# vpc-ccg/freddie

Measured on AMD Instinct MI355X. Metric: reads segmented/sec (whole node), higher is better.
Workload: dtype u32

## Files before the change

### freddie_amd/csrc/seg_common.h

```cpp
#pragma once
#include <hip/hip_runtime.h>
#include <type_traits>
#include <hsa/hsa.h>
#include <hsa/hsa_ext_amd.h>
#include <chrono>
#include <algorithm>
#include <atomic>
#include <mutex>
#include <cmath>
#include <cstdarg>
#include <cstdio>
#include <cstdlib>
#include <cstring>
#include <string>
#include <vector>

#include "freddie_seg.h"

namespace fseg {


typedef long long i64;

typedef unsigned long long u64;
// ... 344 lines not shown
#define FSEG_VAL(x) (pass ? __dmul_rn(__dsub_rn((x), mu), __dsub_rn((x), mu)) : (x))
    for (int t0 = 0; t0 < nl; t0 += 64) {
        int t = t0 + (threadIdx.x >> 3);
        double res = 0.0;
        if (t < nl) {
            const double *b = a + L.leaf_off[t];
            int len = L.leaf_len[t];
            if (len < 8) {
                for (int i = 0; i < len; ++i) res = __dadd_rn(res, FSEG_VAL(b[i]));
            } else {
                int body = len - (len % 8);
                double x[16];
#pragma unroll
                for (int i = 0; i < 16; ++i) x[i] = (8 * i + q < body) ? b[8 * i + q] : 0.0;
                double r = FSEG_VAL(x[0]);
#pragma unroll
                for (int i = 1; i < 16; ++i) if (8 * i + q < body) r = __dadd_rn(r, FSEG_VAL(x[i]));
                r = __dadd_rn(r, __shfl_xor(r, 1));
                r = __dadd_rn(r, __shfl_xor(r, 2));
                r = __dadd_rn(r, __shfl_xor(r, 4));
                res = r;
                for (int i = body; i < len; ++i) res = __dadd_rn(res, FSEG_VAL(b[i]));
            }
        }
        if (t < nl && q == 0) L.node_val[L.leaf_heap[t]] = res;
    }
#undef FSEG_VAL
    __syncthreads();
    double out = 0.0;
    if (m == 8192) {
        if (threadIdx.x < 64) {
            double x = L.node_val[64 + threadIdx.x];
            for (int d = 1; d < 64; d <<= 1) x = __dadd_rn(x, __shfl_xor(x, d));
            out = x;
        }
    } else {
        for (int lvl = 6; lvl >= 0; --lvl) {
            const int i = (1 << lvl) + threadIdx.x;
            if ((int)threadIdx.x < (1 << lvl) && L.node_kind[i] == 2) L.node_val[i] = __dadd_rn(L.node_val[2 * i], L.node_val[2 * i + 1]);
            __syncthreads();
        }
        if (threadIdx.x == 0) out = L.node_val[1];
    }
    return out;
}

constexpr int kThrPartMaxChunks = 128;

__device__ __forceinline__ int wave_emit_values(i64 w0, i64 n_pos, unsigned fm, i64 ex, const double *__restrict__ y, double *v) {
    const int lane = lane_id();
    const u64 lt_mask = (1ULL << lane) - 1ULL;
    u64 rows;
    {
        const u64 lanes_set = __ballot(fm != 0);
        u64 pairs = (lanes_set | (lanes_set >> 1)) & 0x5555555555555555ULL;
        pairs = (pairs | (pairs >> 1)) & 0x3333333333333333ULL;
        pairs = (pairs | (pairs >> 2)) & 0x0f0f0f0f0f0f0f0fULL;
        pairs = (pairs | (pairs >> 4)) & 0x00ff00ff00ff00ffULL;
        pairs = (pairs | (pairs >> 8)) & 0x0000ffff0000ffffULL;
        rows = (pairs | (pairs >> 16)) & 0x00000000ffffffffULL;
    }
    int cnt = 0;
    while (rows) {
        u64 m[8];
        double yv[8];
#pragma unroll
        for (int e = 0; e < 8; ++e) {
            const int q = rows ? (int)__builtin_ctzll(rows) : -1;
            rows = rows ? rows & (rows - 1) : 0;
            const int qq = q < 0 ? 0 : q;
            const unsigned lo = (unsigned)__builtin_amdgcn_readlane((int)fm, 2 * qq);
            const unsigned hi = (unsigned)__builtin_amdgcn_readlane((int)fm, 2 * qq + 1);
            m[e] = q < 0 ? 0 : ((u64)lo | ((u64)hi << 32));
            const i64 i = w0 + qq * 64 + lane;
            yv[e] = y[i < n_pos ? i : n_pos - 1];
        }
#pragma unroll
        for (int e = 0; e < 8; ++e) {
            if (!m[e]) continue;
            if ((m[e] >> lane) & 1ULL) v[ex + cnt + __popcll(m[e] & lt_mask)] = yv[e];
            cnt += __popcll(m[e]);
        }
    }
    return cnt;
}


__device__ __forceinline__ void peak_from(i64 p, i64 last , const double *x, unsigned *flag) {
    const double xi = x[p];
    if (!(x[p - 1] < xi)) return;
    if (x[p + 1] < xi) { set_flag(flag, p); return; }
    if (x[p + 1] == xi) {
        i64 ia = p + 1;
        while (ia < last && x[ia] == xi) ++ia;
        if (x[ia] < xi) set_flag(flag, (p + ia - 1) / 2);
    }
}


struct ProblemArrays {
    int *iv;
    int *start;
    int *n;
    i64 *pair_off;
    i64 *tri_off;
    int *flags;
    int *chain;
    i64 *cov_off;
    int *lane_lo;
    int *lane_n;
};

struct __align__(16) ProbDesc {
    i64 c0;
    i64 pair_off, tri_off, cov_off;
    int n, lane_lo, lane_n;
    int g0;
    int outside;
    int iv;
    int w0;
    int kind;
};

static_assert(sizeof(ProbDesc) == 64, "ProbDesc is one 64-byte record");

__device__ __forceinline__ ProbDesc load_desc(const ProbDesc *d) {
    const uint4 *q = reinterpret_cast<const uint4 *>(d);
    union { uint4 v[4]; ProbDesc p; } u;
    u.v[0] = q[0]; u.v[1] = q[1]; u.v[2] = q[2]; u.v[3] = q[3];
    return u.p;
}


typedef int int4u __attribute__((ext_vector_type(4), aligned(4)));

typedef int int2u __attribute__((ext_vector_type(2), aligned(4)));

__device__ __forceinline__ void load_exons8(const int *p, int (&v)[8]) {
    const int4u a = *reinterpret_cast<const int4u *>(p), b = *reinterpret_cast<const int4u *>(p + 4);
    v[0] = a.x; v[1] = a.y; v[2] = a.z; v[3] = a.w; v[4] = b.x; v[5] = b.y; v[6] = b.z; v[7] = b.w;
}

__device__ __forceinline__ int2 load_exons2(const int *p) {
    const int2u a = *reinterpret_cast<const int2u *>(p);
    return make_int2(a.x, a.y);
}

constexpr size_t kExonPad = 32;

constexpr size_t kLexPad = 64;


__device__ __forceinline__ int uni(int v) { return __builtin_amdgcn_readfirstlane(v); }

__device__ __forceinline__ int wave_id() { return uni((int)(threadIdx.x >> 6)); }

__device__ __forceinline__ ProbDesc load_desc_uniform(const ProbDesc *d) {
    const uint4 *q = reinterpret_cast<const uint4 *>(d);
    union { uint4 v[4]; int w[16]; ProbDesc p; } u;
    u.v[0] = q[0]; u.v[1] = q[1]; u.v[2] = q[2]; u.v[3] = q[3];
#pragma unroll
    for (int i = 0; i < 16; ++i) u.w[i] = uni(u.w[i]);
    return u.p;
}


#ifdef FSEG_DESC_VECTOR
#define FSEG_LOAD_DESC load_desc
#else
#define FSEG_LOAD_DESC load_desc_uniform
#endif

__device__ __forceinline__ i64 wave_excl_scan(i64 v, i64 *total) {
    int lane = lane_id();
    i64 x = v;
    for (int d = 1; d < 64; d <<= 1) {
        i64 y = __shfl_up(x, d);
        if (lane >= d) x += y;
    }
    *total = __shfl(x, 63);
    return x - v;
}


__device__ __forceinline__ int wg_prev_flagged(bool f, int idx, int &carry, int *lds) {
    int lane = lane_id(), wave = threadIdx.x >> 6, nw = (blockDim.x + 63) >> 6;
    u64 mask = __ballot(f);
    __syncthreads();
    if (lane == 0) lds[wave] = mask ? idx + 63 - __clzll((long long)mask) : -1;
    __syncthreads();
    u64 below = mask & ((1ULL << lane) - 1ULL);
    int prev = carry;
    if (below) prev = idx - lane + 63 - __clzll((long long)below);
    else for (int w = wave - 1; w >= 0; --w) if (lds[w] >= 0) { prev = lds[w]; break; }
    for (int w = nw - 1; w >= 0; --w) if (lds[w] >= 0) { carry = lds[w]; break; }
    return prev;
}


__device__ __forceinline__ void window_exons(const int2 *__restrict__ lex, int2 lx, int cp0, int c_last, int *first_rel, int *cnt_out) {
    const int n_ex = lx.y - lx.x;
    int fr = 0, cnt = 0;
    for (int eb = 0; eb < n_ex; eb += 8) {
        int4u x[4];
#pragma unroll
        for (int u = 0; u < 4; ++u) x[u] = *reinterpret_cast<const int4u *>(lex + lx.x + eb + 2 * u);
#pragma unroll
        for (int u = 0; u < 4; ++u) {
            const bool hit0 = eb + 2 * u < n_ex && x[u].y >= cp0 && x[u].x < c_last;
            if (hit0 && cnt == 0) fr = eb + 2 * u;
            cnt += hit0;
            const bool hit1 = eb + 2 * u + 1 < n_ex && x[u].w >= cp0 && x[u].z < c_last;
            if (hit1 && cnt == 0) fr = eb + 2 * u + 1;
            cnt += hit1;
        }
        if (eb + 7 < n_ex && x[3].z >= c_last) break;
    }
    *first_rel = fr; *cnt_out = cnt;
}


constexpr int kRangeThreads = 1024;


constexpr int kProbCols = 9;

__device__ __forceinline__ i64 col_lo(i64 x) { return x & 0xffffffffLL; }

__device__ __forceinline__ i64 col_hi(i64 x) { return (i64)((u64)x >> 32); }

constexpr int kDpSmall = 32;

constexpr int kClsSmall = 16, kClsMid = 32;

struct ProbSizes { i64 v[kProbCols]; };

__device__ __forceinline__ int size_class(int n) { return n <= kClsSmall ? 0 : (n <= kClsMid ? 1 : (n <= kNMax ? 2 : 3)); }

struct ProbSplit { int tiny_max, fuse_lanes; };

enum { kKindArena = 0, kKindTiny = 1, kKindFused = 2, kKindFusedWide = 3 };

__device__ __forceinline__ int prob_kind(int n, int n_lanes, ProbSplit sp) {
    if (n <= sp.tiny_max) return kKindTiny;
    return (n_lanes <= sp.fuse_lanes && n <= kNMax) ? kKindFused : kKindArena;
}

__device__ __forceinline__ ProbSizes prob_sizes(int n, int n_lanes, ProbSplit sp) {
    ProbSizes s;
    for (int q = 0; q < kProbCols; ++q) s.v[q] = 0;
    if (n <= 0) return s;
    const int kind = prob_kind(n, n_lanes, sp);
    if (kind == kKindTiny) { s.v[0] = 1; s.v[8] = 1LL << 32; return s; }
    if (kind == kKindFused) {
        const int c = size_class(n);
        s.v[0] = 1;
        s.v[7] = c == 0 ? 1 : (c == 1 ? (1LL << 32) : 0);
        s.v[8] = c == 2 ? 1 : 0;
        return s;
    }
    i64 chunks = (n_lanes + kLaneChunk - 1) / kLaneChunk;
    const int cls = size_class(n);
    s.v[0] = 1 + (n <= kDpSmall ? (1LL << 32) : 0);
    s.v[1] = (i64)n * (n - 1) / 2; s.v[2] = (i64)n * (n - 1) * (n - 2) / 6;
    s.v[3] = chunks * kLaneChunk * n;
    s.v[4] = cls == 0 ? chunks : (cls == 1 ? chunks << 32 : 0);
    s.v[5] = (cls == 2 ? chunks : 0) + ((n > kDpSmall && n <= kNMax) ? (1LL << 32) : 0);
    s.v[6] = (cls == 3 ? chunks : 0) + (n > kNMax ? (1LL << 32) : 0);
    return s;
}

__device__ __forceinline__ i64 wg_exclusive_scan64(i64 v, i64 *lds , i64 *total) {
    int lane = lane_id(), wave = threadIdx.x >> 6, nw = (blockDim.x + 63) >> 6;
    i64 x = v;
    for (int d = 1; d < 64; d <<= 1) {
        i64 y = __shfl_up(x, d);
        if (lane >= d) x += y;
    }
    __syncthreads();
    if (lane == 63) lds[wave] = x;
    __syncthreads();
    i64 off = 0, tot = 0;
    for (int w = 0; w < nw; ++w) {
        i64 sv = lds[w];
        if (w < wave) off += sv;
        tot += sv;
    }
    *total = tot;
    return off + x - v;
}

constexpr int kProbBlock = 1024;

__device__ __forceinline__ void wg_scan_cols(const ProbSizes &v, ProbSizes &ex, ProbSizes &tot, i64 *lds ) {
    const int lane = lane_id(), wave = threadIdx.x >> 6;
    for (int q = 0; q < kProbCols; ++q) {
        i64 x = v.v[q];
        if (__ballot(x != 0)) {
            for (int d = 1; d < 64; d <<= 1) {
                i64 y = __shfl_up(x, d);
                if (lane >= d) x += y;
            }
        }
        ex.v[q] = x - v.v[q];
        if (lane == 63) lds[wave * kProbCols + q] = x;
    }
// ... 588 lines not shown
```

### freddie_amd/csrc/seg_score_fused.hip

```cpp
#include "seg_kernels.h"

namespace fseg {


#ifndef FSEG_TINY_OCC
#define FSEG_TINY_OCC 5
#endif
__global__ void __launch_bounds__(256, FSEG_TINY_OCC) k_tiny(Status *st, const ProbDesc *desc, i64 prob_cap, int tiny_max, ProblemArrays pr,
                                              const int *cand_y, const longlong2 *lane_ex, const int *ex_ts,
                                              const int *ex_te, const double *h_table, int h_len, double tau, const int2 *thr_tab,
                                              int support, unsigned char *chosen, i64 lb_h, i64 ln_h FSEG_TPARAM) {
    __shared__ u64 planes[4][kTinyPairs][2];
    __shared__ i64 M_s[4][kTinyPairs];
    __shared__ int in_s[4][kTinyPairs];
    __shared__ unsigned out_s[4][kTinyTri + 4];
    __shared__ unsigned char A_s[4][kTinyPairs + 4];
    __shared__ int cy_s[4][kTiny];
    __shared__ unsigned char tri_ijk[kTinyTri][4];
    __shared__ int2 act_w[4][128];
    const int lane = lane_id(), wave = wave_id();
    const u64 lt_mask = (1ULL << lane) - 1ULL;
    if (threadIdx.x < kTinyTri) {
        int t = threadIdx.x, k = 2;
        while ((k + 1) * k * (k - 1) / 6 <= t) ++k;
// ... 80 lines not shown
            int cov[kTiny];
#pragma unroll
            for (int j = 0; j < kTiny; ++j) cov[j] = 0;
            {
                const int2 a = act_w[wave][valid ? lane : 0];
                const int e_end = valid ? a.y : 0;
                for (int e = 0; e < e_end; e += 2) {
                    const int2 ts2 = load_exons2(ex_ts + a.x + e), te2 = load_exons2(ex_te + a.x + e);
                    const int tsa = ts2.x, tea = te2.x, tsb = ts2.y, teb = te2.y;
                    const int a0 = max(tsa, cp0), b0 = tea + 1;
                    const int a1 = max(tsb, cp0), b1 = e + 1 < e_end ? teb + 1 : a1;
#pragma unroll
                    for (int j = 1; j < kTiny; ++j) cov[j] += max(0, min(b0, cj[j]) - a0) + max(0, min(b1, cj[j]) - a1);
                }
            }
            const u64 vmask = __ballot(valid);
            u64 my_yea = 0, my_nay = 0;
#pragma unroll
            for (int j = 1; j < kTiny; ++j) {
#pragma unroll
                for (int i = 0; i < j; ++i) {
                    const int q = j * (j - 1) / 2 + i;
                    if (q < npairs) {
                        const int dd = cov[j] - cov[i];
                        const int hi = __builtin_amdgcn_readlane(hi_q, q), lo = __builtin_amdgcn_readlane(lo_q, q);
                        const u64 y = __ballot(valid && dd >= hi), z = __ballot(valid && dd <= lo);
                        if (lane == q) { my_yea = y; my_nay = z; }
                    }
                }
            }
            if (lane < npairs) {
                amb += (unsigned)__popcll(~(my_yea | my_nay) & vmask);
                planes[wave][lane][0] = my_yea; planes[wave][lane][1] = my_nay;
            }
            int2 keep = make_int2(0, 0);
            if (lane < fill - nv) keep = act_w[wave][64 + lane];
            dp_sync<64>();
            if (lane < fill - nv) act_w[wave][lane] = keep;
            fill -= nv;
            if (lane < ntri) {
                const int qa = tj * (tj - 1) / 2 + ti, qb = tk * (tk - 1) / 2 + tj;
                out += (unsigned)(__popcll(planes[wave][qa][0] & planes[wave][qb][1]) + __popcll(planes[wave][qa][1] & planes[wave][qb][0]));
            }
            dp_sync<64>();
        }
        const int dropped = d.lane_n - n_act;
        if (lane < npairs) in_s[wave][lane] = -(int)((i64)amb + (lo_q < 0 ? (i64)d.outside + dropped : 0));
        if (lane < ntri) out_s[wave][lane] = out;
        dp_sync<64>();
        const int chain = dp_solve_push<64, kTiny>(n, out_s[wave], in_s[wave], M_s[wave], A_s[wave], cy_s[wave], support, chosen + d.c0 FSEG_DARG);
        if (lane == 0) pr.chain[p] = chain;
#ifdef FSEG_SCORE_TIMING
        if (lane == 0) FSEG_PROB_TICK(p, t_prob0, d.lane_n, n_act);
#endif
    }
}

template <int NM, typename V>
__global__ void __launch_bounds__(256, WaveCfg<NM>::kOcc) k_wave(Status *st, const ProbDesc *desc, i64 prob_cap, int list, ProblemArrays pr,
                                                                 const int *__restrict__ cand_y, const int2 *__restrict__ lane_lx, const int2 *__restrict__ lex,
                                                                 const double *h_table, int h_len, double tau, const int2 *__restrict__ thr_tab,
                                                                 int support, unsigned char *chosen, i64 lb_h, i64 ln_h FSEG_TPARAM) {
    using C = WaveCfg<NM>;
    __shared__ WaveLds<NM, V> lds4[4];
    __shared__ unsigned short tri_q[C::kTri + 2];
    const int lane = lane_id(), wave = wave_id();
    WaveLds<NM, V> &L = lds4[wave];
    for (int t = threadIdx.x; t < C::kTri; t += 256) {
        int k = 2;
        while ((k + 1) * k * (k - 1) / 6 <= t) ++k;
        int i, j;
        pair_decode(t - k * (k - 1) * (k - 2) / 6, &i, &j);
        tri_q[t] = (unsigned short)((j * (j - 1) / 2 + i) | ((k * (k - 1) / 2 + j) << 8));
    }
    __syncthreads();
    if (lb_h < 0 && (i64)st->n_prob > prob_cap) return;
#ifdef FSEG_SCORE_TIMING
    __shared__ unsigned long long tick_sink[16];
    unsigned long long *dp_tacc = tick_sink; unsigned long long dt_prev = 0;
#endif
    const i64 list_base = lb_h >= 0 ? lb_h : (list == 3 ? (i64)st->solve_cls[0] + (i64)st->solve_cls[1] + (i64)st->solve_cls[2] : 0);
    const i64 list_n = lb_h >= 0 ? ln_h : (list == 3 ? (i64)st->n_tiny : (i64)st->solve_cls[0]);
    const unsigned aborted = stage_aborted(st);
    for (i64 t = (i64)blockIdx.x + (i64)wave * gridDim.x; t < list_n; t += (i64)gridDim.x * 4) {
#ifdef FSEG_SCORE_TIMING
        const unsigned long long t_prob0 = wall_clock64();
#endif
        const ProbDesc d = FSEG_LOAD_DESC(desc + list_base + t);
        if (aborted) return;
        const int p = d.w0;
        const int n = d.n;
        if (n > NM || n < 3) { if (lane == 0) atomicOr(&st->err, kErrOverflowNm); continue; }
        const int npairs = n * (n - 1) / 2, ntri = n * (n - 1) * (n - 2) / 6;
        int2 lx = lane_lx[d.lane_lo + (lane < d.lane_n ? lane : 0)];
        const int cyv = cand_y[d.c0 + (lane < n ? lane : 0)];
        dp_sync<64>();
        if (lane < n) L.cy[lane] = cyv;
        int hi_q[C::kPSlots], lo_q[C::kPSlots];
        unsigned amb[C::kPSlots], outc[C::kTSlots];
#pragma unroll
        for (int s = 0; s < C::kPSlots; ++s) {
            const int q = s * 64 + lane;
            hi_q[s] = 0x7fffffff; lo_q[s] = -1; amb[s] = 0;
            const unsigned short ij = g_pair_ij[q < npairs ? q : 0];
            const int ci = __shfl(cyv, ij & 255), cjv = __shfl(cyv, ij >> 8);
            if (q < npairs) label_thresholds_tab((i64)cjv - ci + 1, thr_tab, h_table, h_len, tau, &hi_q[s], &lo_q[s]);
        }
#pragma unroll
        for (int s = 0; s < C::kTSlots; ++s) outc[s] = 0;
        const int cp0 = d.g0 + __builtin_amdgcn_readlane(cyv, 0), c_last = d.g0 + __builtin_amdgcn_readlane(cyv, n - 1);
        int cj[NM];
#pragma unroll
        for (int j = 0; j < NM; ++j) cj[j] = j < n ? d.g0 + __builtin_amdgcn_readlane(cyv, j) : cp0;
        for (int l0 = 0; l0 < d.lane_n;) {
            const bool in = l0 + lane < d.lane_n;
            if (l0 > 0) lx = lane_lx[d.lane_lo + l0 + (in ? lane : 0)];
            const int base = uni(lx.x) & ~1;
            const u64 fm = __ballot(in && lx.y - base <= kStageCap);
            const int m = ~fm == 0 ? 64 : (int)__builtin_ctzll(~fm);
            if (m == 0) { if (lane == 0) atomicOr(&st->err, kErrWaveStage); break; }
            const int total = __builtin_amdgcn_readlane(lx.y, m - 1) - base;
            {
                const int last2 = total & ~1;
                int4 sv[kStageCap / 128];
#pragma unroll
                for (int u = 0; u < kStageCap / 128; ++u) {
                    const int i = 2 * lane + 128 * u;
                    sv[u] = *reinterpret_cast<const int4 *>(lex + base + (i < last2 ? i : last2));
                }
#pragma unroll
                for (int u = 0; u < kStageCap / 128; ++u) {
                    const int i = 2 * lane + 128 * u;
                    if (i < total) *reinterpret_cast<int4 *>(&L.stage[i]) = sv[u];
                }
            }
            dp_sync<64>();
            const bool valid = lane < m;
            const u64 vmask = m == 64 ? ~0ULL : ((1ULL << m) - 1ULL);
            const int ea = valid ? lx.x - base : 0, eb = valid ? lx.y - base : 0;
            int first = ea, cnt = 0;
            for (int e = ea; e < eb; e += 4) {
                int2 x[4];
#pragma unroll
                for (int u = 0; u < 4; ++u) x[u] = L.stage[e + u];
#pragma unroll
                for (int u = 0; u < 4; ++u) {
                    const bool hit = e + u < eb && x[u].y >= cp0 && x[u].x < c_last;
                    if (hit && cnt == 0) first = e + u;
                    cnt += hit;
                }
                if (x[3].x >= c_last) break;
            }
            int cov[NM];
#pragma unroll
            for (int j = 0; j < NM; ++j) cov[j] = 0;
            for (int e = 0; e < cnt; e += 2) {
                const int2 xa = L.stage[first + e], xb = L.stage[first + e + 1];
                const int a0 = max(xa.x, cp0), b0 = xa.y + 1;
                const int a1 = max(xb.x, cp0), b1 = e + 1 < cnt ? xb.y + 1 : a1;
#pragma unroll
                for (int j = 1; j < NM; ++j)
                    if (j < n) cov[j] += max(0, min(b0, cj[j]) - a0) + max(0, min(b1, cj[j]) - a1);
            }
            unsigned yl[C::kPSlots], yh[C::kPSlots], zl[C::kPSlots], zh[C::kPSlots];
#pragma unroll
            for (int s = 0; s < C::kPSlots; ++s) { yl[s] = 0; yh[s] = 0; zl[s] = 0; zh[s] = 0; }
            static_for<1, NM>([&](auto jc) {
                constexpr int j = decltype(jc)::value;
                if (j < n) {
                    static_for<0, j>([&](auto ic) {
                        constexpr int i = decltype(ic)::value;
                        constexpr int q = j * (j - 1) / 2 + i, s = q >> 6, ql = q & 63;
                        const int dd = cov[j] - cov[i];
                        const int hi = __builtin_amdgcn_readlane(hi_q[s], ql), lo = __builtin_amdgcn_readlane(lo_q[s], ql);
                        const u64 y = __ballot(dd >= hi) & vmask, z = __ballot(dd <= lo) & vmask;
                        write_lane<ql>(yl[s], (unsigned)y); write_lane<ql>(yh[s], (unsigned)(y >> 32));
                        write_lane<ql>(zl[s], (unsigned)z); write_lane<ql>(zh[s], (unsigned)(z >> 32));
                    });
                }
            });
#pragma unroll
            for (int s = 0; s < C::kPSlots; ++s) {
                const int q = s * 64 + lane;
                if (q < npairs) {
                    amb[s] += (unsigned)(__popc(~(yl[s] | zl[s]) & (unsigned)vmask) + __popc(~(yh[s] | zh[s]) & (unsigned)(vmask >> 32)));
                    L.planes[q] = make_uint4(yl[s], yh[s], zl[s], zh[s]);
                }
            }
            dp_sync<64>();
#pragma unroll
            for (int s = 0; s < C::kTSlots; ++s) {
                const int tt = s * 64 + lane;
                if (tt < ntri) {
                    const unsigned tq = tri_q[tt];
                    const uint4 a = L.planes[tq & 255], b = L.planes[tq >> 8];
                    outc[s] += (unsigned)(__popc((a.x & b.z) | (a.z & b.x)) + __popc((a.y & b.w) | (a.w & b.y)));
                }
            }
            dp_sync<64>();
            l0 += m;
        }
#pragma unroll
        for (int s = 0; s < C::kPSlots; ++s) {
            const int q = s * 64 + lane;
            if (q < npairs) L.in[q] = -(int)((i64)amb[s] + (lo_q[s] < 0 ? (i64)d.outside : 0));
        }
#pragma unroll
        for (int s = 0; s < C::kTSlots; ++s) {
            const int tt = s * 64 + lane;
            if (tt < ntri) L.out[tt] = outc[s];
        }
        dp_sync<64>();
        const int chain = dp_solve_push<64, NM>(n, L.out, L.in, L.M, L.A, L.cy, support, chosen + d.c0 FSEG_DARG);
        if (lane == 0) pr.chain[p] = chain;
#ifdef FSEG_SCORE_TIMING
        if (lane == 0) FSEG_PROB_TICK(p, t_prob0, d.lane_n, d.lane_n);
#endif
    }
}


__global__ void __launch_bounds__(64) k_gate(Status *st, int which, unsigned grid, unsigned max_ticks) {
    const unsigned want = grid;
    const unsigned long long t0 = wall_clock64();
    const unsigned *ctr = which == 2 ? &st->gate_wide : &st->gate;
    while (__hip_atomic_load(ctr, __ATOMIC_RELAXED, __HIP_MEMORY_SCOPE_AGENT) < want && wall_clock64() - t0 < max_ticks && !stage_aborted(st))
        __builtin_amdgcn_s_sleep(16);
}

__global__ void __launch_bounds__(64) k_wait_word(Status *st, const unsigned *words, unsigned mask, unsigned gen, unsigned max_ticks) {
    const int lane = lane_id();
    const bool mine = lane < 32 && ((mask >> lane) & 1u);
    const unsigned *w = words + (mine ? lane : 0);
    const unsigned long long t0 = wall_clock64();
    bool ok = false;
    for (;;) {
        ok = !mine || gen_reached(__hip_atomic_load(w, __ATOMIC_ACQUIRE, __HIP_MEMORY_SCOPE_AGENT), gen);
        if (__all(ok) || wall_clock64() - t0 >= max_ticks) break;
        __builtin_amdgcn_s_sleep(8);
    }
    if (!__all(ok) && lane == 0) {
        __hip_atomic_store(&st->sync_abort, 1u, __ATOMIC_RELEASE, __HIP_MEMORY_SCOPE_AGENT);
        atomicOr(&st->err, kErrSyncTimeout);
    }
}

__global__ void __launch_bounds__(64) k_signal(unsigned *word, unsigned gen) {
    if (threadIdx.x == 0) __hip_atomic_store(word, gen, __ATOMIC_RELEASE, __HIP_MEMORY_SCOPE_AGENT);
}

__global__ void __launch_bounds__(64) k_probe_wait(const unsigned *word, unsigned gen, unsigned *result, unsigned max_ticks) {
    const unsigned long long t0 = wall_clock64();
    bool ok = false;
    for (;;) {
        ok = gen_reached(__hip_atomic_load(word, __ATOMIC_ACQUIRE, __HIP_MEMORY_SCOPE_AGENT), gen);
        if (ok || wall_clock64() - t0 >= max_ticks) break;
        __builtin_amdgcn_s_sleep(8);
    }
    if (threadIdx.x == 0) __hip_atomic_store(result, ok ? 1u : 2u, __ATOMIC_RELEASE, __HIP_MEMORY_SCOPE_AGENT);
}


template <int NM, typename OutT, typename V, int T>
__global__ void __launch_bounds__(T) k_dpw(Status *st, int nm, i64 list_base, i64 list_n, ProblemArrays pr, const ProbDesc *desc,
                                            const unsigned char *dpx, i64 dpx_stride,
                                            int support, unsigned char *chosen, const int *__restrict__ wide_items FSEG_TPARAM) {
    extern __shared__ __align__(16) unsigned char smem[];
    const int lane = T == 64 ? lane_id() : (int)threadIdx.x;
    if ((i64)blockIdx.x >= list_n) return;
    const unsigned aborted = stage_aborted(st);
    if (wide_items && aborted) return;
    const i64 t = wide_items ? (i64)uni(wide_items[list_base + blockIdx.x]) : (i64)blockIdx.x;
#ifdef FSEG_SCORE_TIMING
    const unsigned long long t_dp0 = wall_clock64();
#endif
    const unsigned char *slot = dpx + t * dpx_stride;
    const ProbDesc d = FSEG_LOAD_DESC(desc + list_base + t);
    const int n = d.n;
    if (aborted) return;
    if (n > nm || n > NM || n < 3 || d.lane_n > kFuseLanesWide) return;
    if ((d.kind == kKindFusedWide) != (sizeof(OutT) != 1)) return;
    const int npairs = n * (n - 1) / 2, ntri = n * (n - 1) * (n - 2) / 6;
    const int rt_pairs = nm * (nm - 1) / 2;
    V *M = reinterpret_cast<V *>(smem);
    int *in_s = reinterpret_cast<int *>(smem + (((size_t)rt_pairs * sizeof(V) + 15) & ~(size_t)15));
    unsigned char *A = reinterpret_cast<unsigned char *>(in_s) + (((size_t)rt_pairs * 4 + 15) & ~(size_t)15);
    OutT *out_s = reinterpret_cast<OutT *>(A + (((size_t)rt_pairs + 15) & ~(size_t)15));
    {
        const int *g_in = reinterpret_cast<const int *>(slot + kDpxHeader);
        for (int q = lane; q < npairs; q += T) { in_s[q] = g_in[q]; A[q] = (unsigned char)(g_pair_ij[q] >> 8); }
        const uint4 *g_out = reinterpret_cast<const uint4 *>(slot + kDpxHeader + dpx_in_bytes(nm));
        uint4 *l_out = reinterpret_cast<uint4 *>(out_s);
        const int n16 = (ntri * (int)sizeof(OutT) + 15) / 16;
        constexpr int kInFlight = T == 64 ? 8 : 2;
        for (int x0 = 0; x0 < n16; x0 += T * kInFlight) {
            uint4 v[kInFlight];
#pragma unroll
            for (int u = 0; u < kInFlight; ++u) { const int x = x0 + u * T + lane; v[u] = g_out[x < n16 ? x : 0]; }
#pragma unroll
            for (int u = 0; u < kInFlight; ++u) { const int x = x0 + u * T + lane; if (x < n16) l_out[x] = v[u]; }
        }
    }
    dp_sync<T>();
#ifdef FSEG_SCORE_TIMING
    __shared__ unsigned long long tick_sink[16];
    unsigned long long *dp_tacc = tick_sink; unsigned long long dt_prev = 0;
#endif
    int chain;
    if constexpr (T == 64) chain = dp_solve_wave<NM>(n, out_s, in_s, M, A, support, chosen + d.c0 FSEG_DARG);
    else chain = dp_solve_push<T, NM, OutT, V, true>(n, out_s, in_s, M, A, nullptr, support, chosen + d.c0 FSEG_DARG);
    if (lane == 0) pr.chain[d.w0] = chain;
#ifdef FSEG_SCORE_TIMING
    if (lane == 0 && (size_t)d.w0 < kTaccProbs) { unsigned long long *r_ = tacc + 16 + 4 * kTaccProbs + 4 * (size_t)d.w0; r_[0] = wall_clock64() - t_dp0; r_[1] = (unsigned long long)hw_where() << 32; r_[3] = t_dp0; }
#endif
}

// ... 24 lines not shown
```

### freddie_amd/csrc/seg_solve.h

```cpp
#pragma once
#include "seg_kernels.h"

namespace fseg {

template <int NM, typename CntT, typename V, bool SPLIT>
__global__ void __launch_bounds__(SolveCfg<NM>::kThreads, SolveCfg<NM>::kMinBlocks) k_solve(Status *st, int cls, int nm, i64 lb_h, i64 ln_h, ProblemArrays pr,
                                                                  const ProbDesc *desc, i64 prob_cap, const int *cand_y,
                                                                  const int2 *__restrict__ lane_lx, const int2 *__restrict__ lex,
                                                                  const double *h_table, int h_len, double tau, const int2 *thr_tab,
                                                                  int support, unsigned char *chosen,
                                                                  unsigned char *dpx, i64 dpx_stride,
                                                                  const int *__restrict__ wide_items FSEG_TPARAM) {
    using C = SolveCfg<NM>;
    constexpr int T = C::kThreads, NR = C::kRanges;
    constexpr int PACK = 4 / (int)sizeof(CntT);
    extern __shared__ __align__(16) unsigned char smem[];
    __shared__ int cy_s[NM + 4];
    __shared__ int iend_s[NM + 4];
    __shared__ int2 act_s[sizeof(CntT) == 1 ? kFuseLanes + 1 : kFuseLanesWide + 1];
    __shared__ int act_wave[T / 64];
    const int rt_pairs = nm * (nm - 1) / 2;
    constexpr int rt_stride = NM + 1;
    uint4 *planes = reinterpret_cast<uint4 *>(smem);
    unsigned *cov = reinterpret_cast<unsigned *>(smem + (size_t)rt_pairs * 16);
    const unsigned shared_b = (unsigned)rt_pairs * 16 + (unsigned)(kSub * rt_stride * 4);
    CntT *cnt = reinterpret_cast<CntT *>(smem + ((shared_b + 15) & ~15u));
    V *M = reinterpret_cast<V *>(smem);
    int *in_s = reinterpret_cast<int *>(M + rt_pairs);
    unsigned char *A = reinterpret_cast<unsigned char *>(in_s + rt_pairs);
    constexpr bool kWaveDp = NM <= 32 || sizeof(V) == 4;
    if (NM == kNMax && threadIdx.x == 0) { atomicAdd(&st->gate, 1u); if (sizeof(CntT) != 1) atomicAdd(&st->gate_wide, 1u); }
    if (lb_h < 0 && (i64)st->n_prob > prob_cap) return;
    const i64 list_base = lb_h >= 0 ? lb_h : (cls <= 0 ? 0 : (cls == 1 ? (i64)st->solve_cls[0] : (i64)st->solve_cls[0] + (i64)st->solve_cls[1]));
    const i64 list_n = lb_h >= 0 ? ln_h : (cls < 0 ? (i64)st->solve_cls[0] + (i64)st->solve_cls[1] + (i64)st->solve_cls[2] : (i64)st->solve_cls[cls]);
    const int r_lane = threadIdx.x & 63, w_rng = wave_id();
    const bool own_wg = (i64)gridDim.x >= list_n;
    const unsigned aborted = stage_aborted(st);
#ifdef FSEG_SCORE_TIMING
    __shared__ unsigned long long tick_sink[16];
    const bool timed = (int)tacc[15] == cls;
    unsigned long long *tk = timed ? tacc : tick_sink;
    unsigned long long *dp_tacc = tk; unsigned long long dt_prev = wall_clock64();
#define FSEG_STICK(i) FSEG_DTICK(i)
#else
#define FSEG_STICK(i)
#endif
    for (i64 tt = blockIdx.x; tt < list_n; tt += gridDim.x) {
#ifdef FSEG_SCORE_TIMING
        const unsigned long long t_prob0 = wall_clock64();
#endif
        if (wide_items && aborted) return;
        const i64 t = wide_items ? (i64)uni(wide_items[list_base + tt]) : tt;
        const ProbDesc d = FSEG_LOAD_DESC(desc + list_base + t);
        if (aborted) return;
        const int p = d.w0;
        const int n = d.n;
        __syncthreads();
        FSEG_STICK(0);
        unsigned char *slot = SPLIT ? dpx + t * dpx_stride : nullptr;
        if (n > nm || n > NM) { if (threadIdx.x == 0) atomicOr(&st->err, kErrOverflowNm); continue; }
        if ((d.kind == kKindFusedWide) != (sizeof(CntT) != 1)) continue;
        if (d.lane_n > kFuseLanesWide) { if (threadIdx.x == 0) atomicOr(&st->err, kErrNeedWideDp); continue; }
        const int npairs = n * (n - 1) / 2, ntri = n * (n - 1) * (n - 2) / 6;
        const int *cy = cand_y + d.c0;
        for (int j = threadIdx.x; j < n; j += T) cy_s[j] = cy[j];
        {
            uint4 *z = reinterpret_cast<uint4 *>(cnt);
            for (int x = threadIdx.x; x < (ntri * (int)sizeof(CntT) + 15) / 16; x += T) z[x] = make_uint4(0, 0, 0, 0);
        }
        __syncthreads();
        int pi[C::kSlots], pj[C::kSlots], th_hi[C::kSlots], th_lo[C::kSlots];
        unsigned amb_acc[C::kSlots];
#pragma unroll
        for (int s = 0; s < C::kSlots; ++s) {
            const int q = s * T + threadIdx.x;
            amb_acc[s] = 0; pi[s] = 0; pj[s] = 1; th_hi[s] = 0x7fffffff; th_lo[s] = -1;
            if (q < npairs) {
                const unsigned short ij = g_pair_ij[q];
                pi[s] = ij & 255; pj[s] = ij >> 8;
                label_thresholds_tab((i64)cy_s[pj[s]] - cy_s[pi[s]] + 1, thr_tab, h_table, h_len, tau, &th_hi[s], &th_lo[s]);
            }
        }
        if (threadIdx.x < n) {
            int j = threadIdx.x, lim = cy_s[j] - 5, lo = 0, hi = j;
            while (lo < hi) { int mid = (lo + hi) >> 1; if (cy_s[mid] <= lim) lo = mid + 1; else hi = mid; }
            iend_s[j] = lo;
        }
        const int cp0 = d.g0 + cy_s[0], c_last = d.g0 + cy_s[n - 1];
        int n_act = 0;
        for (int l0 = 0; l0 < d.lane_n; l0 += T) {
            const int l = l0 + (int)threadIdx.x;
            const bool in = l < d.lane_n;
#ifdef FSEG_ABLATE_COV
            const int2 ex = make_int2(0, 0);
            int first_rel = 0, cnt = (l % 3) != 2;
#else
            const int2 ex = lane_lx[d.lane_lo + (in ? l : 0)];
            int first_rel, cnt;
            window_exons(lex, ex, cp0, c_last, &first_rel, &cnt);
#endif
            const int first = ex.x + first_rel;
            const bool act = in && cnt > 0;
            const u64 m = __ballot(act);
            if ((threadIdx.x & 63) == 0) act_wave[threadIdx.x >> 6] = __popcll(m);
            __syncthreads();
            int base = n_act, tot = 0;
            for (int w2 = 0; w2 < T / 64; ++w2) { const int v = act_wave[w2]; if (w2 < (int)(threadIdx.x >> 6)) base += v; tot += v; }
            {
                constexpr int kActCap = sizeof(CntT) == 1 ? kFuseLanes + 1 : kFuseLanesWide + 1;
                const int slot = base + __popcll(m & ((1ULL << (threadIdx.x & 63)) - 1ULL));
                if (act && slot < kActCap) act_s[slot] = make_int2(first, cnt);
            }
            n_act += tot;
            __syncthreads();
        }
        if (sizeof(CntT) == 1 && n_act > kFuseLanes) { if (threadIdx.x == 0) atomicOr(&st->err, kErrWideMissed); continue; }
        FSEG_STICK(1);
        constexpr int kCovJ = (NM - 1 + NR - 1) / NR;
        const int ja = 1 + (int)((i64)(n - 1) * w_rng / NR), jb = 1 + (int)((i64)(n - 1) * (w_rng + 1) / NR);
        int cjv[kCovJ];
#pragma unroll
        for (int u = 0; u < kCovJ; ++u) cjv[u] = ja + u < jb ? d.g0 + cy_s[ja + u] : cp0;
        for (int r0 = 0; r0 < n_act; r0 += kSub) {
            int n_valid = n_act - r0;
            if (n_valid > kSub) n_valid = kSub;
            {
                const bool valid = r_lane < n_valid;
                const int2 a = act_s[r0 + (valid ? r_lane : 0)];
                int acc[kCovJ];
#pragma unroll
                for (int u = 0; u < kCovJ; ++u) acc[u] = 0;
#ifdef FSEG_ABLATE_COV
                const int e_end = 0;
#else
                const int e_end = valid ? a.y : 0;
#endif
                for (int e = 0; e < e_end; e += 4) {
                    const int4u x01 = *reinterpret_cast<const int4u *>(lex + a.x + e), x23 = *reinterpret_cast<const int4u *>(lex + a.x + e + 2);
                    {
                        const int a0 = max(x01.x, cp0), b0 = x01.y + 1;
                        const int a1 = max(x01.z, cp0), b1 = e + 1 < e_end ? x01.w + 1 : a1;
#pragma unroll
                        for (int v = 0; v < kCovJ; ++v) acc[v] += max(0, min(b0, cjv[v]) - a0) + max(0, min(b1, cjv[v]) - a1);
                    }
                    if (e + 2 < e_end) {
                        const int a0 = max(x23.x, cp0), b0 = x23.y + 1;
                        const int a1 = max(x23.z, cp0), b1 = e + 3 < e_end ? x23.w + 1 : a1;
#pragma unroll
                        for (int v = 0; v < kCovJ; ++v) acc[v] += max(0, min(b0, cjv[v]) - a0) + max(0, min(b1, cjv[v]) - a1);
                    }
                }
#pragma unroll
                for (int u = 0; u < kCovJ; ++u) if (ja + u < jb) cov[r_lane * rt_stride + ja + u] = (unsigned)acc[u];
                if (w_rng == 0) cov[r_lane * rt_stride] = 0;
            }
            lds_barrier();
            FSEG_STICK(2);
            const int nv1 = n_valid - 32;
            const unsigned valid0 = n_valid >= 32 ? 0xffffffffu : (n_valid > 0 ? ~(0xffffffffu >> n_valid) : 0u);
            const unsigned valid1 = nv1 >= 32 ? 0xffffffffu : (nv1 > 0 ? ~(0xffffffffu >> nv1) : 0u);
#pragma unroll
            for (int s = 0; s < C::kSlots; ++s) {
                const int q = s * T + threadIdx.x;
                if (q < npairs) {
                    const int i = pi[s], j = pj[s], hi = th_hi[s], lo = th_lo[s];
                    unsigned y0 = 0, z0 = 0, y1 = 0, z1 = 0;
#define FSEG_SHIFT_IN(acc, cmp, a, b) asm("v_cmp_" cmp "_i32_e32 vcc, %1, %2\n\tv_addc_co_u32_e32 %0, vcc, %0, %0, vcc" : "+v"(acc) : "v"(a), "v"(b) : "vcc")
                    if (n_valid >= 32) {
#pragma unroll
                        for (int b = 0; b < 32; ++b) {
                            int dd = (int)(cov[b * rt_stride + j] - cov[b * rt_stride + i]);
                            FSEG_SHIFT_IN(y0, "ge", dd, hi);
                            FSEG_SHIFT_IN(z0, "le", dd, lo);
                        }
                    } else {
                        for (int b = 0; b < n_valid; ++b) {
                            int dd = (int)(cov[b * rt_stride + j] - cov[b * rt_stride + i]);
                            FSEG_SHIFT_IN(y0, "ge", dd, hi);
                            FSEG_SHIFT_IN(z0, "le", dd, lo);
                        }
                        y0 <<= 32 - n_valid; z0 <<= 32 - n_valid;
                    }
                    if (nv1 >= 32) {
#pragma unroll
                        for (int b = 0; b < 32; ++b) {
                            int dd = (int)(cov[(32 + b) * rt_stride + j] - cov[(32 + b) * rt_stride + i]);
                            FSEG_SHIFT_IN(y1, "ge", dd, hi);
                            FSEG_SHIFT_IN(z1, "le", dd, lo);
                        }
                    } else if (nv1 > 0) {
                        for (int b = 0; b < nv1; ++b) {
                            int dd = (int)(cov[(32 + b) * rt_stride + j] - cov[(32 + b) * rt_stride + i]);
                            FSEG_SHIFT_IN(y1, "ge", dd, hi);
                            FSEG_SHIFT_IN(z1, "le", dd, lo);
                        }
                        y1 <<= 32 - nv1; z1 <<= 32 - nv1;
                    }
#undef FSEG_SHIFT_IN
                    y0 &= valid0; z0 &= valid0; y1 &= valid1; z1 &= valid1;
                    planes[q] = make_uint4(y0, y1, z0, z1);
                    amb_acc[s] += __popc(~(y0 | z0) & valid0) + __popc(~(y1 | z1) & valid1);
                }
            }
            lds_barrier();
            FSEG_STICK(3);
#pragma unroll
            for (int s = 0; s < C::kSlots; ++s) {
                const int r = s * T + threadIdx.x;
                if (r >= npairs) continue;
                const int m = pj[s], x = pi[s];
                const int j = n - 1 - m, kk = j + 1 + x;
                if (j == 0 || cy_s[kk] - cy_s[j] < 5) continue;
                const uint4 B = planes[kk * (kk - 1) / 2 + j];
                if ((B.x | B.y | B.z | B.w) == 0) continue;
                const int tbase = kk * (kk - 1) * (kk - 2) / 6 + j * (j - 1) / 2;
                const int abase = j * (j - 1) / 2;
                const int i_end = iend_s[j];
#define FSEG_TRI_CNT(Av) (HALF ? __popc(((Av).x & B.z) | ((Av).z & B.x)) \
                               : __popc(((Av).x & B.z) | ((Av).z & B.x)) + __popc(((Av).y & B.w) | ((Av).w & B.y)))
                CntT *o = cnt + tbase;
                auto row = [&](auto half_c) {
                    constexpr bool HALF = decltype(half_c)::value;
                    int i = 0;
                    for (; i < i_end && ((tbase + i) & (PACK - 1)); ++i) {
                        const uint4 Av = planes[abase + i];
                        o[i] = (CntT)(o[i] + FSEG_TRI_CNT(Av));
                    }
                    for (; i + PACK <= i_end; i += PACK) {
                        unsigned add = 0;
#pragma unroll
                        for (int u = 0; u < PACK; ++u) { const uint4 Av = planes[abase + i + u]; add |= (unsigned)FSEG_TRI_CNT(Av) << (8 * (int)sizeof(CntT) * u); }
                        *reinterpret_cast<unsigned *>(o + i) += add;
                    }
                    for (; i < i_end; ++i) {
                        const uint4 Av = planes[abase + i];
                        o[i] = (CntT)(o[i] + FSEG_TRI_CNT(Av));
                    }
                };
                if (n_valid <= 32) row(std::true_type{}); else row(std::false_type{});
#undef FSEG_TRI_CNT
            }
            lds_barrier();
            FSEG_STICK(4);
        }
        int in_val[C::kSlots];
#pragma unroll
        for (int s = 0; s < C::kSlots; ++s) in_val[s] = -(int)((i64)amb_acc[s] + (th_lo[s] < 0 ? (i64)d.outside + (d.lane_n - n_act) : 0));
        __syncthreads();
        if constexpr (SPLIT) {
            int *g_in = reinterpret_cast<int *>(slot + kDpxHeader);
#pragma unroll
            for (int s = 0; s < C::kSlots; ++s) {
                const int q = s * T + threadIdx.x;
                if (q < npairs) {
                    const bool dead = cy_s[pj[s]] - cy_s[pi[s]] < 5 && !(pi[s] == 0 && pj[s] == n - 1);
                    g_in[q] = dead ? kDeadPair : in_val[s];
                }
            }
            {
                uint4 *g_out = reinterpret_cast<uint4 *>(slot + kDpxHeader + dpx_in_bytes(nm));
                const uint4 *l_out = reinterpret_cast<const uint4 *>(cnt);
                for (int x = threadIdx.x; x < (ntri * (int)sizeof(CntT) + 15) / 16; x += T) g_out[x] = l_out[x];
            }
            FSEG_STICK(9);
        } else if constexpr (kWaveDp) {
#pragma unroll
            for (int s = 0; s < C::kSlots; ++s) {
                const int q = s * T + threadIdx.x;
                if (q < npairs) {
                    const bool dead = cy_s[pj[s]] - cy_s[pi[s]] < 5 && !(pi[s] == 0 && pj[s] == n - 1);
                    in_s[q] = dead ? kDeadPair : in_val[s];
                    A[q] = (unsigned char)pj[s];
                }
            }
            __syncthreads();
            FSEG_STICK(9);
            if (w_rng != 0) { if (own_wg) return; continue; }
#ifdef FSEG_ABLATE_DP
            if (own_wg) return;
#endif
            const int chain = dp_solve_wave<NM>(n, cnt, in_s, M, A, support, chosen + d.c0 FSEG_DARG);
            if (threadIdx.x == 0) pr.chain[p] = chain;
        } else {
#pragma unroll
        for (int s = 0; s < C::kSlots; ++s) { const int q = s * T + threadIdx.x; if (q < npairs) in_s[q] = in_val[s]; }
        __syncthreads();
        FSEG_STICK(9);
        const int chain = dp_solve_push<T, NM>(n, cnt, in_s, M, A, cy_s, support, chosen + d.c0 FSEG_DARG);
        if (threadIdx.x == 0) pr.chain[p] = chain;
        }
#ifdef FSEG_SCORE_TIMING
        if (threadIdx.x == 0) FSEG_PROB_TICK(p, t_prob0, d.lane_n, n_act);
#endif
    }
#undef FSEG_STICK
}

}
```

Before: 577.6 million.

## Use med3 clamp for coverage and packed 16-bit pair comparisons in solve

Rewrites the coverage accumulation as sum of med3(c, a, b) minus the summed starts, replacing max/min/sub chains with a single v_med3 per term in both the tiny and solve kernels. When the column span fits in 15 bits, k_solve stores coverage as interleaved 16-bit halves and builds the y/z pair bitplanes with packed 16-bit subtracts and sign extraction, handling two reads per instruction. This is meant to cut VALU work in the pair-classification stage. It adds a row-permuted LDS layout and a new bit-order mapping for valid masks, which must stay consistent with the later triple-counting stage. It also adds ablation macros.

```diff
diff --git a/freddie_amd/csrc/seg_common.h b/freddie_amd/csrc/seg_common.h
--- a/freddie_amd/csrc/seg_common.h
+++ b/freddie_amd/csrc/seg_common.h
@@ -520,6 +520,11 @@
 
 
 __device__ __forceinline__ int uni(int v) { return __builtin_amdgcn_readfirstlane(v); }
+__device__ __forceinline__ int clamp_to(int c, int a, int b) {
+    int r;
+    asm("v_med3_i32 %0, %1, %2, %3" : "=v"(r) : "v"(c), "v"(a), "v"(b));
+    return r;
+}
 
 __device__ __forceinline__ int wave_id() { return uni((int)(threadIdx.x >> 6)); }
 
diff --git a/freddie_amd/csrc/seg_score_fused.hip b/freddie_amd/csrc/seg_score_fused.hip
--- a/freddie_amd/csrc/seg_score_fused.hip
+++ b/freddie_amd/csrc/seg_score_fused.hip
@@ -256,6 +256,7 @@
                 if (x[3].x >= c_last) break;
             }
             int cov[NM];
+            unsigned sub_a = 0;
 #pragma unroll
             for (int j = 0; j < NM; ++j) cov[j] = 0;
             for (int e = 0; e < cnt; e += 2) {
@@ -264,8 +265,12 @@
                 const int a1 = max(xb.x, cp0), b1 = e + 1 < cnt ? xb.y + 1 : a1;
 #pragma unroll
                 for (int j = 1; j < NM; ++j)
-                    if (j < n) cov[j] += max(0, min(b0, cj[j]) - a0) + max(0, min(b1, cj[j]) - a1);
-            }
+                    if (j < n) cov[j] = (int)((unsigned)cov[j] + (unsigned)clamp_to(cj[j], a0, b0) + (unsigned)clamp_to(cj[j], a1, b1));
+                sub_a += (unsigned)a0 + (unsigned)a1;
+            }
+#pragma unroll
+            for (int j = 1; j < NM; ++j)
+                if (j < n) cov[j] = (int)((unsigned)cov[j] - sub_a);
             unsigned yl[C::kPSlots], yh[C::kPSlots], zl[C::kPSlots], zh[C::kPSlots];
 #pragma unroll
             for (int s = 0; s < C::kPSlots; ++s) { yl[s] = 0; yh[s] = 0; zl[s] = 0; zh[s] = 0; }
diff --git a/freddie_amd/csrc/seg_solve.h b/freddie_amd/csrc/seg_solve.h
--- a/freddie_amd/csrc/seg_solve.h
+++ b/freddie_amd/csrc/seg_solve.h
@@ -2,6 +2,27 @@
 #include "seg_kernels.h"
 
 namespace fseg {
+
+constexpr int kPk16Window = 32767;
+typedef short pk16_t __attribute__((ext_vector_type(2)));
+typedef unsigned short pk16u_t __attribute__((ext_vector_type(2)));
+__device__ __forceinline__ unsigned pk16_sub(unsigned a, unsigned b) {
+    return __builtin_bit_cast(unsigned, (pk16_t)(__builtin_bit_cast(pk16_t, a) - __builtin_bit_cast(pk16_t, b)));
+}
+__device__ __forceinline__ unsigned pk16_sign(unsigned a) { return __builtin_bit_cast(unsigned, (pk16u_t)(__builtin_bit_cast(pk16u_t, a) >> 15)); }
+__device__ __forceinline__ unsigned pk16_dup(int v) { return ((unsigned)v & 0xffffu) * 0x10001u; }
+__device__ __forceinline__ void pk16_step(unsigned cj, unsigned ci, unsigned hi_m1, unsigned lo_p1, unsigned &y, unsigned &z) {
+    const unsigned dd = pk16_sub(cj, ci);
+    y = (y << 1) | pk16_sign(pk16_sub(hi_m1, dd));
+    z = (z << 1) | pk16_sign(pk16_sub(dd, lo_p1));
+    asm("" : "+v"(y), "+v"(z));
+}
+
+__device__ __forceinline__ unsigned pk16_valid(int nv) {
+    if (nv >= 32) return 0xffffffffu;
+    if (nv <= 16) return (1u << nv) - 1u;
+    return 0xffffu | (0xffff0000u & ~(0xffffffffu >> (nv - 16)));
+}
 
 template <int NM, typename CntT, typename V, bool SPLIT>
 __global__ void __launch_bounds__(SolveCfg<NM>::kThreads, SolveCfg<NM>::kMinBlocks) k_solve(Status *st, int cls, int nm, i64 lb_h, i64 ln_h, ProblemArrays pr,
@@ -71,6 +92,11 @@
         __syncthreads();
         int pi[C::kSlots], pj[C::kSlots], th_hi[C::kSlots], th_lo[C::kSlots];
         unsigned amb_acc[C::kSlots];
+#ifdef FSEG_NO_PK16
+        const bool pk16 = false;
+#else
+        const bool pk16 = uni(cy_s[n - 1] - cy_s[0]) < kPk16Window;
+#endif
 #pragma unroll
         for (int s = 0; s < C::kSlots; ++s) {
             const int q = s * T + threadIdx.x;
@@ -127,7 +153,7 @@
             {
                 const bool valid = r_lane < n_valid;
                 const int2 a = act_s[r0 + (valid ? r_lane : 0)];
-                int acc[kCovJ];
+                unsigned acc[kCovJ], sub_a = 0;
 #pragma unroll
                 for (int u = 0; u < kCovJ; ++u) acc[u] = 0;
 #ifdef FSEG_ABLATE_COV
@@ -141,22 +167,62 @@
                         const int a0 = max(x01.x, cp0), b0 = x01.y + 1;
                         const int a1 = max(x01.z, cp0), b1 = e + 1 < e_end ? x01.w + 1 : a1;
 #pragma unroll
-                        for (int v = 0; v < kCovJ; ++v) acc[v] += max(0, min(b0, cjv[v]) - a0) + max(0, min(b1, cjv[v]) - a1);
+                        for (int v = 0; v < kCovJ; ++v) acc[v] += (unsigned)clamp_to(cjv[v], a0, b0) + (unsigned)clamp_to(cjv[v], a1, b1);
+                        sub_a += (unsigned)a0 + (unsigned)a1;
                     }
                     if (e + 2 < e_end) {
                         const int a0 = max(x23.x, cp0), b0 = x23.y + 1;
                         const int a1 = max(x23.z, cp0), b1 = e + 3 < e_end ? x23.w + 1 : a1;
 #pragma unroll
-                        for (int v = 0; v < kCovJ; ++v) acc[v] += max(0, min(b0, cjv[v]) - a0) + max(0, min(b1, cjv[v]) - a1);
-                    }
-                }
-#pragma unroll
-                for (int u = 0; u < kCovJ; ++u) if (ja + u < jb) cov[r_lane * rt_stride + ja + u] = (unsigned)acc[u];
-                if (w_rng == 0) cov[r_lane * rt_stride] = 0;
+                        for (int v = 0; v < kCovJ; ++v) acc[v] += (unsigned)clamp_to(cjv[v], a0, b0) + (unsigned)clamp_to(cjv[v], a1, b1);
+                        sub_a += (unsigned)a0 + (unsigned)a1;
+                    }
+                }
+#pragma unroll
+                for (int u = 0; u < kCovJ; ++u) acc[u] -= sub_a;
+                if (pk16) {
+                    unsigned short *cov16 = reinterpret_cast<unsigned short *>(cov) + ((((r_lane >> 5) << 4) | (r_lane & 15)) * rt_stride) * 2 + ((r_lane >> 4) & 1);
+#pragma unroll
+                    for (int u = 0; u < kCovJ; ++u) if (ja + u < jb) cov16[(ja + u) * 2] = (unsigned short)acc[u];
+                    if (w_rng == 0) cov16[0] = 0;
+                } else {
+#pragma unroll
+                    for (int u = 0; u < kCovJ; ++u) if (ja + u < jb) cov[r_lane * rt_stride + ja + u] = (unsigned)acc[u];
+                    if (w_rng == 0) cov[r_lane * rt_stride] = 0;
+                }
             }
             lds_barrier();
             FSEG_STICK(2);
-            const int nv1 = n_valid - 32;
+            const int nv0 = n_valid < 32 ? n_valid : 32, nv1 = n_valid - nv0;
+            if (pk16) {
+                const unsigned valid0 = pk16_valid(nv0), valid1 = pk16_valid(nv1);
+#pragma unroll
+                for (int s = 0; s < C::kSlots; ++s) {
+                    const int q = s * T + threadIdx.x;
+                    if (q < npairs) {
+                        const int i = pi[s], j = pj[s];
+                        const unsigned hi_m1 = pk16_dup(min(max(th_hi[s], 0), 32767) - 1), lo_p1 = pk16_dup(min(max(th_lo[s], -1), 32766) + 1);
+                        unsigned y0 = 0, z0 = 0, y1 = 0, z1 = 0;
+#ifndef FSEG_ABLATE_PAIRS
+                        auto word = [&](const unsigned *rows, int nv, unsigned &y, unsigned &z) {
+                            if (nv >= 16) {
+#pragma unroll
+                                for (int w = 0; w < 16; ++w) pk16_step(rows[w * rt_stride + j], rows[w * rt_stride + i], hi_m1, lo_p1, y, z);
+                            } else if (nv > 0) {
+                                for (int w = 0; w < nv; ++w) pk16_step(rows[w * rt_stride + j], rows[w * rt_stride + i], hi_m1, lo_p1, y, z);
+                            }
+                        };
+                        word(cov, nv0, y0, z0);
+                        word(cov + 16 * rt_stride, nv1, y1, z1);
+#else
+                        y0 = hi_m1; z0 = ~hi_m1; y1 = lo_p1; z1 = ~lo_p1 & (unsigned)(i + j);
+#endif
+                        y0 &= valid0; z0 &= valid0; y1 &= valid1; z1 &= valid1;
+                        planes[q] = make_uint4(y0, y1, z0, z1);
+                        amb_acc[s] += nv1 > 0 ? __popc(~(y0 | z0) & valid0) + __popc(~(y1 | z1) & valid1) : __popc(~(y0 | z0) & valid0);
+                    }
+                }
+            } else {
             const unsigned valid0 = n_valid >= 32 ? 0xffffffffu : (n_valid > 0 ? ~(0xffffffffu >> n_valid) : 0u);
             const unsigned valid1 = nv1 >= 32 ? 0xffffffffu : (nv1 > 0 ? ~(0xffffffffu >> nv1) : 0u);
 #pragma unroll
@@ -165,6 +231,7 @@
                 if (q < npairs) {
                     const int i = pi[s], j = pj[s], hi = th_hi[s], lo = th_lo[s];
                     unsigned y0 = 0, z0 = 0, y1 = 0, z1 = 0;
+#ifndef FSEG_ABLATE_PAIRS
 #define FSEG_SHIFT_IN(acc, cmp, a, b) asm("v_cmp_" cmp "_i32_e32 vcc, %1, %2\n\tv_addc_co_u32_e32 %0, vcc, %0, %0, vcc" : "+v"(acc) : "v"(a), "v"(b) : "vcc")
                     if (n_valid >= 32) {
 #pragma unroll
@@ -197,17 +264,24 @@
                         y1 <<= 32 - nv1; z1 <<= 32 - nv1;
                     }
 #undef FSEG_SHIFT_IN
+#else
+                    y0 = (unsigned)hi; z0 = ~(unsigned)hi; y1 = (unsigned)lo; z1 = ~(unsigned)lo & (unsigned)(i + j);
+#endif
                     y0 &= valid0; z0 &= valid0; y1 &= valid1; z1 &= valid1;
                     planes[q] = make_uint4(y0, y1, z0, z1);
                     amb_acc[s] += __popc(~(y0 | z0) & valid0) + __popc(~(y1 | z1) & valid1);
                 }
             }
+            }
             lds_barrier();
             FSEG_STICK(3);
 #pragma unroll
             for (int s = 0; s < C::kSlots; ++s) {
                 const int r = s * T + threadIdx.x;
                 if (r >= npairs) continue;
+#ifdef FSEG_ABLATE_TRI
+                continue;
+#endif
                 const int m = pj[s], x = pi[s];
                 const int j = n - 1 - m, kk = j + 1 + x;
                 if (j == 0 || cy_s[kk] - cy_s[j] < 5) continue;
```

Result: no change. 580.9 million (median of 6 runs) (+0.6%).
